# cvjena/semantic-embeddings

Hardware: AMD Instinct MI355X
Metric: retrieval_Mpairs_per_sec (higher is better)
Workload: dtype f32

## Files before the change

semantic-embeddings_amd/csrc/pdist_mfma.hip:

```cpp
#include "se_common.h"
#include <stdlib.h>

namespace se {

typedef float f32x16 __attribute__((ext_vector_type(16)));
typedef float f32x4 __attribute__((ext_vector_type(4)));

constexpr int PD_BM = 128, PD_BN = 128, PD_BK = 64;
constexpr int PD_THREADS = 512;
constexpr int PD_WAVES = PD_THREADS / 64;
constexpr int PD_WROWS = PD_BM / (PD_WAVES / 2);
constexpr int PD_MI = PD_WROWS / 32;
constexpr int PD_LD = PD_BK + 4;
constexpr int PD_SP = PD_BN + 4;
constexpr int PD_SR = (PD_BM * PD_SP <= (PD_BM + PD_BN) * PD_LD) ? PD_BM : PD_BM / 2;
static_assert(PD_SR * PD_SP <= (PD_BM + PD_BN) * PD_LD, "epilogue stage must fit in the operand LDS");
constexpr int PD_GROUP_M = 16;
constexpr int PD_MAX_KB = 16;
constexpr int PD_WGS_PER_CU = 2;
constexpr int PD_F4R = PD_BK / 4;
constexpr int PD_RPP = PD_THREADS / PD_F4R;
constexpr int PD_NLOAD = PD_BM / PD_RPP;
constexpr int64_t PD_MAX_LD = (int64_t)1 << 23;

static_assert(PD_MAX_KB == SE_MAX_KB, "KBlocks capacity");

__device__ __forceinline__ float mask_f(float x, bool keep)
{
    return __uint_as_float(__float_as_uint(x) & (keep ? 0xFFFFFFFFu : 0u));
}

template <bool VEC>
__device__ __forceinline__ void pd_load(float4 (&v)[PD_NLOAD], const float *__restrict__ src, uint32_t ld, int64_t row0,
                                        int64_t nrows, int64_t k0, int64_t kend)
// ... 105 lines not shown
    const uint32_t ldo4 = ldo * 4u;
    float4 cn = make_float4(0.f, 0.f, 0.f, 0.f);
    if (EUC) cn = *(const float4 *)&coln[c4];
#pragma unroll
    for (int p = 0; p < PD_SR / RPP; p++) {
        const int row = p * RPP + r0;
        float4 v = *(const float4 *)&stage[row * PD_SP + c4];
        if (EUC) {
            const float rn = rown[row];
            v = make_float4(fmaf(-2.0f, v.x, rn + cn.x), fmaf(-2.0f, v.y, rn + cn.y), fmaf(-2.0f, v.z, rn + cn.z), fmaf(-2.0f, v.w, rn + cn.w));
        }
        if (dry) { asm volatile("" ::"v"(v.x), "v"(v.y), "v"(v.z), "v"(v.w)); continue; }
        float *dp = (float *)(gb + ((uint32_t)row * ldo4 + (uint32_t)c4 * 4u));
        if (fast) {
            if (nt) __builtin_nontemporal_store((f32x4){v.x, v.y, v.z, v.w}, (f32x4 *)dp);
            else *(float4 *)dp = v;
        } else if (row < nrows) {
            if (c4 < ncols) dp[0] = v.x;
            if (c4 + 1 < ncols) dp[1] = v.y;
            if (c4 + 2 < ncols) dp[2] = v.z;
            if (c4 + 3 < ncols) dp[3] = v.w;
        }
    }
}

template <int METRIC>
__device__ __forceinline__ float pd_finish(float v, float sa, float sb)
{
    if (METRIC == SE_METRIC_COSINE) return -v;
    if (METRIC == SE_METRIC_EUCLID) return (sa + sb) - 2.0f * v;
    return v;
}

constexpr int PDF_VEC_A = 1, PDF_VEC_B = 2, PDF_VEC_O = 4, PDF_NO_STORE = 8, PDF_NO_MFMA = 16, PDF_STAGGER = 32, PDF_PLAIN_ST = 64, PDF_NO_GSTORE = 128;

template <int METRIC, bool MULTI_KB, bool SYM, bool VEC, int EPI>
__global__ __launch_bounds__(PD_THREADS, (PD_WAVES / 4) * PD_WGS_PER_CU) void pdist_kernel(
    const float *__restrict__ A, uint32_t lda, const float *__restrict__ Bm, uint32_t ldb,
    const float *__restrict__ sqa, const float *__restrict__ sqb, int64_t Q, int64_t N, int64_t D,
    KBlocks kbs, int nchunks, float *__restrict__ out, uint32_t ldo, int tiles_m, int tiles_n, int64_t ntiles, int flags,
    unsigned long long *prof, FusedArgs fa)
{
    static_assert(EPI != EPI_GROUPMIN || !SYM, "the sample pass walks the general tile order");
    extern __shared__ __attribute__((aligned(16))) float smem[];
    float *sA = smem;
    float *sB = smem + PD_BM * PD_LD;
    constexpr bool EUC_OUT = METRIC == SE_METRIC_EUCLID && EPI == EPI_STORE;
    [[maybe_unused]] float *sN = smem + (PD_BM + PD_BN) * PD_LD;
    typedef __attribute__((address_space(1))) const void pd_gptr_t;
    typedef __attribute__((address_space(3))) void pd_lptr_t;

    const int64_t b = blockIdx.x, G = gridDim.x;
    const int64_t xcd = b & 7, qq = ntiles >> 3, rr = ntiles & 7;
    const int64_t band_beg = (xcd < rr) ? xcd * (qq + 1) : rr * (qq + 1) + (xcd - rr) * qq;
    const int64_t band_len = qq + (xcd < rr ? 1 : 0);
    const int64_t wg_in_xcd = b >> 3, wgs_per_xcd = (G + 7 - xcd) >> 3;
    const int64_t my_tiles = (band_len > wg_in_xcd) ? (band_len - wg_in_xcd + wgs_per_xcd - 1) / wgs_per_xcd : 0;
    if (my_tiles == 0) return;
    if (flags & PDF_STAGGER) {
        const int slot = (int)((b >> 3) & 3);
        for (int i = 0; i < slot * 2; i++) __builtin_amdgcn_s_sleep(127);
    }

    const int lane = lane_id(), wave = threadIdx.x >> 6;
    const int wm = wave >> 1, wn = wave & 1;
    const int col = lane & 31, hi = lane >> 5;
    const bool vec_o = flags & PDF_VEC_O;
    const bool nt = !(flags & PDF_PLAIN_ST);

    constexpr int NB = 2 * PD_MI;
    f32x16 acc[NB], tot[NB];
#pragma unroll
    for (int j = 0; j < NB; j++)
#pragma unroll
        for (int r = 0; r < 16; r++) { acc[j][r] = 0.f; if (MULTI_KB) tot[j][r] = 0.f; }

    const float *pa = sA + (wm * PD_WROWS + col) * PD_LD + hi * (PD_BK / 2);
    const float *pb0 = sB + (wn * 64 + col) * PD_LD + hi * (PD_BK / 2);
    const float *pb1 = pb0 + 32 * PD_LD;

    float4 ra[PD_NLOAD], rb[PD_NLOAD];
    int64_t m0, n0, k0, kend;
    bool closes_kb;
    pd_tile_coords<SYM>((uint32_t)(band_beg + wg_in_xcd), tiles_m, tiles_n, m0, n0);
    pd_chunk(0, kbs, MULTI_KB, D, k0, kend, closes_kb);
#define PD_FETCH()                              \
    pd_load<VEC>(ra, A, lda, m0, Q, k0, kend);  \
    pd_load<VEC>(rb, Bm, ldb, n0, N, k0, kend);
    PD_FETCH()
    bool first_kb = true;

#ifdef SE_TUNING
    uint64_t t_acc[12] = {0, 0, 0, 0, 0, 0, 0, 0, 0, 0, 0, 0}, t_last = prof ? __builtin_amdgcn_s_memtime() : 0;
#define PD_T(i) if (prof) { const uint64_t now = __builtin_amdgcn_s_memtime(); t_acc[i] += now - t_last; t_last = now; }
#else
#define PD_T(i)
#endif
    const int64_t total = my_tiles * nchunks;
    int c = 0;
    uint32_t tile_i = 0;
    int64_t cur_m0 = m0, cur_n0 = n0;
    int kc = (int)((kend - k0 < PD_BK) ? (kend - k0) : PD_BK);
    bool cur_closes = closes_kb;
    pd_store(sA, ra, (int)((Q - cur_m0 < PD_BM) ? (Q - cur_m0) : PD_BM), kc);
    pd_store(sB, rb, (int)((N - cur_n0 < PD_BN) ? (N - cur_n0) : PD_BN), kc);
    wg_barrier();
#pragma unroll 1
    for (int64_t it = 0; it < total; it++) {
        PD_T(2)
        const bool last_chunk = (c + 1 == nchunks);
        const bool have_next = it + 1 < total;
        if (EUC_OUT && last_chunk) {
            const int w_ = threadIdx.x >> 6;
            if (w_ < (PD_BM + PD_BN) / 64) {
                const int t_ = threadIdx.x & (PD_BM - 1);
                const bool rows_ = w_ < PD_BM / 64;
                const int64_t i_ = rows_ ? (cur_m0 + t_ < Q ? cur_m0 + t_ : Q - 1) : (cur_n0 + t_ < N ? cur_n0 + t_ : N - 1);
                const float *src_ = (rows_ ? sqa : sqb) + i_;
                __builtin_amdgcn_global_load_lds((pd_gptr_t *)src_, (pd_lptr_t *)(sN + w_ * 64), 4, 0, 0);
            }
        }
        if (have_next) {
            const int nc = last_chunk ? 0 : c + 1;
            if (nc == 0) pd_tile_coords<SYM>((uint32_t)(band_beg + wg_in_xcd) + (tile_i + 1u) * (uint32_t)wgs_per_xcd, tiles_m, tiles_n, m0, n0);
            pd_chunk(nc, kbs, MULTI_KB, D, k0, kend, closes_kb);
            PD_FETCH()
        }

        PD_T(3)
        const int steps = (flags & PDF_NO_MFMA) ? 0 : ((kc + 1) >> 1);
        const int full = steps & ~3;
#define PD_STEP(C)                                                                                \
    _Pragma("unroll") for (int mi = 0; mi < PD_MI; mi++) {                                        \
        acc[mi * 2] = __builtin_amdgcn_mfma_f32_32x32x2f32(a4[mi].C, b0.C, acc[mi * 2], 0, 0, 0);         \
        acc[mi * 2 + 1] = __builtin_amdgcn_mfma_f32_32x32x2f32(a4[mi].C, b1.C, acc[mi * 2 + 1], 0, 0, 0); \
    }
#define PD_READ(S)                                                                                \
    float4 a4[PD_MI];                                                                             \
    _Pragma("unroll") for (int mi = 0; mi < PD_MI; mi++) a4[mi] = *(const float4 *)(pa + mi * 32 * PD_LD + (S)); \
    const float4 b0 = *(const float4 *)(pb0 + (S));                                               \
    const float4 b1 = *(const float4 *)(pb1 + (S));
        for (int s = 0; s < full; s += 4) {
            PD_READ(s)
            PD_STEP(x) PD_STEP(y) PD_STEP(z) PD_STEP(w)
        }
        if (steps & 3) {
            PD_READ(full)
            PD_STEP(x)
            if ((steps & 3) > 1) { PD_STEP(y) }
            if ((steps & 3) > 2) { PD_STEP(z) }
        }
#undef PD_READ
#undef PD_STEP

        PD_T(4)
        {
#pragma unroll
            for (int i = 0; i < PD_NLOAD; i++) {
                asm volatile("" : "+v"(ra[i].x), "+v"(ra[i].y), "+v"(ra[i].z), "+v"(ra[i].w));
                asm volatile("" : "+v"(rb[i].x), "+v"(rb[i].y), "+v"(rb[i].z), "+v"(rb[i].w));
            }
        }
        if (MULTI_KB && cur_closes) {
#pragma unroll
            for (int j = 0; j < NB; j++)
#pragma unroll
                for (int r = 0; r < 16; r++) {
                    tot[j][r] = first_kb ? acc[j][r] : (tot[j][r] + acc[j][r]);
                    acc[j][r] = 0.f;
                }
            first_kb = false;
        }

        if (last_chunk) {
            if (EUC_OUT) asm volatile("s_waitcnt vmcnt(0)" ::: "memory");
            if (flags & PDF_NO_STORE) {
#pragma unroll
                for (int j = 0; j < NB; j++)
#pragma unroll
                    for (int r = 0; r < 16; r++) asm volatile("" ::"v"(acc[j][r]));
            } else if (EPI != EPI_STORE) {
                const int rows_here = (int)((Q - cur_m0 < PD_BM) ? (Q - cur_m0) : PD_BM);
                const int cols_here = (int)((N - cur_n0 < PD_BN) ? (N - cur_n0) : PD_BN);
                const bool full_rows = rows_here == PD_BM;
                const int lr0 = wm * PD_WROWS + 4 * hi;
#define PD_FVAL(MI_, J, R)                                                                                                   \
    pd_finish<METRIC>(MULTI_KB ? tot[(MI_) * 2 + (J)][R] : acc[(MI_) * 2 + (J)][R],                                            \
                      METRIC == SE_METRIC_EUCLID ? fsa[((R) & 3) + 4 * ((R) >> 2)] : 0.f, sbq)
                if (EPI == EPI_GROUPMIN) {
#pragma unroll
                    for (int mi = 0; mi < PD_MI; mi++) {
                        float fsa[16];
                        if (METRIC == SE_METRIC_EUCLID) {
#pragma unroll
                            for (int r = 0; r < 16; r++) {
                                const int lr = lr0 + mi * 32 + (r & 3) + 8 * (r >> 2);
                                fsa[r] = sqa[(cur_m0 + (lr < rows_here ? lr : rows_here - 1)) * fa.sqa_stride];
                            }
                        }
#pragma unroll
                        for (int j = 0; j < 2; j++) {
                            const int lc = wn * 64 + j * 32 + col;
                            const bool qok = lc < cols_here;
                            const int64_t qg = cur_n0 + (qok ? lc : cols_here - 1);
                            const float sbq = METRIC == SE_METRIC_EUCLID ? sqb[qg] : 0.f;
                            float m = __builtin_inff();
                            bool any = false;
// ... 176 lines not shown
#pragma unroll
                    for (int h = 0; h < PD_BN / PD_SR; h++) {
                        wg_barrier();
                        PD_T(6)
                        if ((wn * 64) / PD_SR == h) {
#pragma unroll
                            for (int mi = 0; mi < PD_MI; mi++)
#pragma unroll
                                for (int j = 0; j < 2; j++)
#pragma unroll
                                    for (int g = 0; g < 4; g++)
                                        *(float4 *)&smem[(wn * 64 - h * PD_SR + j * 32 + col) * PD_SP + lr0 + mi * 32 + 8 * g] =
                                            make_float4(PD_VAL(mi, j, 4 * g), PD_VAL(mi, j, 4 * g + 1), PD_VAL(mi, j, 4 * g + 2), PD_VAL(mi, j, 4 * g + 3));
                        }
                        PD_T(7)
                        wg_barrier();
                        PD_T(8)
                        pd_stream_rows<EUC_OUT>(smem, out + ((cur_n0 + h * PD_SR) * (int64_t)ldo + cur_m0), ldo, cols_here - h * PD_SR, rows_here, fast, nt,
                                                flags & PDF_NO_GSTORE, sN + PD_BM + h * PD_SR, sN);
                        PD_T(9)
                    }
                }
#undef PD_VAL
            }
#pragma unroll
            for (int j = 0; j < NB; j++)
#pragma unroll
                for (int r = 0; r < 16; r++) acc[j][r] = 0.f;
            first_kb = true;
            PD_T(5)
        }
        wg_barrier();
        PD_T(0)
        if (have_next) {
            cur_m0 = m0; cur_n0 = n0;
            kc = (int)((kend - k0 < PD_BK) ? (kend - k0) : PD_BK);
            cur_closes = closes_kb;
            pd_store(sA, ra, (int)((Q - cur_m0 < PD_BM) ? (Q - cur_m0) : PD_BM), kc);
            pd_store(sB, rb, (int)((N - cur_n0 < PD_BN) ? (N - cur_n0) : PD_BN), kc);
        }
        PD_T(1)
        wg_barrier();
        c = last_chunk ? 0 : c + 1;
        tile_i += last_chunk ? 1u : 0u;
    }
#ifdef SE_TUNING
    if (prof && threadIdx.x == 0)
        for (int i = 0; i < 12; i++) atomicAdd(&prof[i], (unsigned long long)t_acc[i]);
#endif
#undef PD_T
#undef PD_FETCH
}

template <int METRIC, bool MULTI, bool SYM, bool VEC, int EPI = EPI_STORE>
static int launch_pdist3(const float *a, int64_t lda, const float *b, int64_t ldb, const float *sqa, const float *sqb,
                         int64_t q, int64_t n, int64_t d, const KBlocks &kbs, float *out, int64_t ldo, hipStream_t s,
                         const FusedArgs &fa = FusedArgs{nullptr, 0, nullptr, nullptr, nullptr, 0, 1})
{
    const int tiles_m = (int)((q + PD_BM - 1) / PD_BM), tiles_n = (int)((n + PD_BN - 1) / PD_BN);
    const int64_t ntiles = SYM ? ((int64_t)tiles_n * (tiles_n + 1) / 2) : ((int64_t)tiles_m * tiles_n);
    const size_t lds = ((size_t)(PD_BM + PD_BN) * PD_LD + (METRIC == SE_METRIC_EUCLID && EPI == EPI_STORE ? PD_BM + PD_BN : 0)) * sizeof(float);
    if (ntiles >= ((int64_t)1 << 31) || (int64_t)PD_GROUP_M * tiles_n >= ((int64_t)1 << 31) || (SYM && tiles_n > 65535))
        return fail(SE_ERR_UNSUPPORTED, "se_pairwise_dist: %lld output tiles exceed the 32-bit tile counter -- split the call", (long long)ntiles);
    int flags = 0;
    if ((lda % 4 == 0) && ((((uintptr_t)a) & 15) == 0)) flags |= PDF_VEC_A;
    if ((ldb % 4 == 0) && ((((uintptr_t)b) & 15) == 0)) flags |= PDF_VEC_B;
    if ((ldo % 4 == 0) && ((((uintptr_t)out) & 15) == 0)) flags |= PDF_VEC_O;
    flags |= PDF_STAGGER;
    if (kTuning) {
        static const int tune = [] {
            int f = 0;
            if (const char *e = tuning_env("SE_PD_ABLATE")) { const int a = atoi(e); f |= (a & 3) * PDF_NO_STORE; if (a & 4) f |= PDF_NO_GSTORE; }
            if (tuning_env("SE_PD_NOSTAGGER")) f |= 1 << 30;
            if (tuning_env("SE_PD_PLAIN_ST")) f |= PDF_PLAIN_ST;
            return f;
        }();
        flags |= tune & ~(1 << 30);
        if (tune & (1 << 30)) flags &= ~PDF_STAGGER;
    }
    int nchunks = 0;
    for (int i = 0; i < kbs.n; i++) nchunks += (kbs.len[i] + PD_BK - 1) / PD_BK;
    int64_t grid = (int64_t)num_cus() * PD_WGS_PER_CU;
    grid = grid / 8 * 8;
    if (grid > ntiles) grid = ntiles;
    if (grid < 1) grid = 1;
    auto kern = pdist_kernel<METRIC, MULTI, SYM, VEC, EPI>;
    SE_HIP_CHECK(hipFuncSetAttribute((const void *)kern, hipFuncAttributeMaxDynamicSharedMemorySize, (int)lds));
    static const bool profile = tuning_env("SE_PD_PROFILE") != nullptr;
    unsigned long long *prof = nullptr;
    if (profile) {
        SE_HIP_CHECK(hipMalloc((void **)&prof, 12 * sizeof(unsigned long long)));
        SE_HIP_CHECK(hipMemsetAsync(prof, 0, 12 * sizeof(unsigned long long), s));
    }
    hipLaunchKernelGGL(kern, dim3((unsigned)grid), dim3(PD_THREADS), lds, s, a, (uint32_t)lda, b, (uint32_t)ldb, sqa, sqb, q, n,
                       d, kbs, nchunks, out, (uint32_t)ldo, tiles_m, tiles_n, ntiles, flags, prof, fa);
    SE_LAUNCH_CHECK();
    if (profile) {
        unsigned long long h[12];
        SE_HIP_CHECK(hipStreamSynchronize(s));
        SE_HIP_CHECK(hipMemcpy(h, prof, sizeof(h), hipMemcpyDeviceToHost));
        SE_HIP_CHECK(hipFree(prof));
        static const char *names[12] = {"wait-barrier", "stage-operands", "barrier", "prefetch-issue", "mfma", "epilogue-rest",
                                        "epi-barrier-in", "epi-stage-write", "epi-barrier", "epi-stream-out", "-", "-"};
        double tot = 0;
        for (int i = 0; i < 12; i++) tot += (double)h[i];
        fprintf(stderr, "[se_pairwise_dist profile] sym=%d grid=%lld tiles=%lld:", (int)SYM, (long long)grid, (long long)ntiles);
        for (int i = 0; i < 10; i++) fprintf(stderr, " %s %.1f%%", names[i], 100.0 * (double)h[i] / tot);
        fprintf(stderr, "  (%.0f cycles per tile per workgroup)\n", tot / (double)ntiles);
    }
    return SE_OK;
}

template <int METRIC, bool MULTI, bool SYM>
static int launch_pdist2(const float *a, int64_t lda, const float *b, int64_t ldb, const float *sqa, const float *sqb,
                         int64_t q, int64_t n, int64_t d, const KBlocks &kbs, float *out, int64_t ldo, hipStream_t s)
{
    bool vec = (lda % 4 == 0) && ((((uintptr_t)a) & 15) == 0) && (ldb % 4 == 0) && ((((uintptr_t)b) & 15) == 0);
    int64_t beg = 0;
    for (int i = 0; i < kbs.n; i++) { if (beg & 3) vec = false; beg += kbs.len[i]; }
    return vec ? launch_pdist3<METRIC, MULTI, SYM, true>(a, lda, b, ldb, sqa, sqb, q, n, d, kbs, out, ldo, s)
               : launch_pdist3<METRIC, MULTI, SYM, false>(a, lda, b, ldb, sqa, sqb, q, n, d, kbs, out, ldo, s);
}

template <int METRIC>
static int launch_pdist(const float *a, int64_t lda, const float *b, int64_t ldb, const float *sqa, const float *sqb,
                        int64_t q, int64_t n, int64_t d, const KBlocks &kbs, bool multi, float *out, int64_t ldo,
                        hipStream_t s)
{
    const bool sym = (a == b) && (lda == ldb) && (q == n) && (METRIC != SE_METRIC_EUCLID || sqa == sqb) && n > PD_BN;
    if (sym) return multi ? launch_pdist2<METRIC, true, true>(a, lda, b, ldb, sqa, sqb, q, n, d, kbs, out, ldo, s)
                          : launch_pdist2<METRIC, false, true>(a, lda, b, ldb, sqa, sqb, q, n, d, kbs, out, ldo, s);
    return multi ? launch_pdist2<METRIC, true, false>(a, lda, b, ldb, sqa, sqb, q, n, d, kbs, out, ldo, s)
                 : launch_pdist2<METRIC, false, false>(a, lda, b, ldb, sqa, sqb, q, n, d, kbs, out, ldo, s);
// ... 89 lines not shown
```

semantic-embeddings_amd/csrc/rank_rows.hip:

```cpp
#include "se_common.h"
#include <stdlib.h>
#include <atomic>
#include <type_traits>

namespace se {

constexpr int RK_THREADS = 512;
constexpr int RK_WAVES = RK_THREADS / WAVE;
constexpr int RK_ITEMS = 16;
constexpr int RK_TILE = RK_THREADS * RK_ITEMS;
constexpr int RK_WCHUNK = RK_TILE / RK_WAVES;
constexpr int RK_NB = 256;

struct RankLds {
    uint32_t gbase[4][RK_NB];
    uint32_t wcnt[RK_WAVES][RK_NB];
    uint32_t tile_start[RK_NB];
    uint32_t wave_tot[RK_WAVES];
    uint32_t tkeys[RK_TILE];
    uint32_t tidx[RK_TILE];
};

__device__ __forceinline__ uint32_t wave_excl_scan(uint32_t v, uint32_t &total)
{
// ... 399 lines not shown
    constexpr int BITS = HWORD ? RR_HW_BITS : 8;
    constexpr int NB = 1 << BITS;
    constexpr int NPASS = (32 + BITS - 1) / BITS;
    constexpr int CNT_WORDS = HWORD ? NB / 2 : NB;
    constexpr bool WIDE = HWORD && ((size_t)RR_THREADS * ITEMS * sizeof(uint16_t) >= (size_t)RR_WAVES * RR_WIDE_WORDS * sizeof(uint32_t));
    constexpr bool IMG = WIDE && VAR == 3;
    constexpr bool RAWKEYS = IMG || (WIDE && VAR == 2);
    static_assert(VAR != 3 || (WIDE && ITEMS <= RR_IMG_MAX_ITEMS && !SEG), "image path: long-row instantiations with room for the tag plane");
    uint32_t *wcnt = reinterpret_cast<uint32_t *>(rr_raw);
    uint32_t *wave_tot = reinterpret_cast<uint32_t *>(rr_raw + rr_region0_bytes<ITEMS, HWORD, VAR>());
    uint16_t *xbuf = reinterpret_cast<uint16_t *>(wave_tot + 32);
    [[maybe_unused]] uint8_t *tagb = rr_raw;
    [[maybe_unused]] uint32_t *wlist = reinterpret_cast<uint32_t *>(rr_raw + (size_t)RR_THREADS * ITEMS + 32);
    [[maybe_unused]] uint32_t *ictl = wave_tot + 24;
    const int tid = threadIdx.x, lane = tid & 63, wave = tid >> 6;
    [[maybe_unused]] const int wave_s = __builtin_amdgcn_readfirstlane(wave);
    const int wpos0 = wave * (ITEMS * WAVE) + lane;
    const uint32_t xb = lds_off(xbuf);
    const uint32_t rb = xb + 2u * (uint32_t)wpos0;
    static_assert(rr_region0_bytes<ITEMS, HWORD, VAR>() % 16 == 0 && (ITEMS * WAVE * sizeof(uint16_t)) % 8 == 0, "transposed reads need 8-byte aligned addresses");
    [[maybe_unused]] const uint32_t rt = xb + 2u * (uint32_t)(wave * (ITEMS * WAVE)) + rr_tr_lane_off((uint32_t)lane);
#define RR_DST(IR) (xb + (((IR) & 0xFFFFu) << 1))
    auto row_ptr = [&](int64_t v) -> const float * {
        if constexpr (SEG) return pdist + (v >> seg.shift) * ldp + (v & ((1 << seg.shift) - 1)) * (int64_t)seg.seg_n;
        else return pdist + v * ldp;
    };
    auto row_len = [&](int64_t v) -> int {
        if constexpr (SEG) {
            const int rest = N - (int)(v & ((1 << seg.shift) - 1)) * seg.seg_n;
            return rest < seg.seg_n ? rest : seg.seg_n;
        } else return N;
    };
    uint32_t t_acc[12] = {0, 0, 0, 0, 0, 0, 0, 0, 0, 0, 0, 0}, t_last = PROF ? (uint32_t)__builtin_amdgcn_s_memtime() : 0;
#define RR_T(i) if constexpr (PROF) { const uint32_t now = (uint32_t)__builtin_amdgcn_s_memtime(); t_acc[i] += now - t_last; t_last = now; } else { asm volatile("" ::: "memory"); __builtin_amdgcn_sched_barrier(0); }

    uint32_t key[ITEMS], ir[ITEMS];
    __amdgpu_buffer_rsrc_t ld_rsrc;
    uint32_t ld_voff = 0;
    uint64_t ring[RR_RING / 2];
#define RR_LOAD_ONE(DROW, WPOS, S, NN)                                                                               \
    {                                                                                                                 \
        if ((S) % 16 == 0) {                                                                                          \
            if ((S) == 0) {                                                                                           \
                ld_rsrc = __builtin_amdgcn_make_buffer_rsrc(const_cast<float *>(DROW), 0, (NN) * 4, 0x00020000);     \
                ld_voff = (uint32_t)(WPOS) * 4u;                                                                      \
            } else ld_voff += 4096u;                                                                                  \
            opaque(ld_voff);                                                                                          \
        }                                                                                                             \
        key[S] = (uint32_t)__builtin_amdgcn_raw_buffer_load_b32(ld_rsrc, (int)ld_voff + ((S) % 16) * 256, 0, 0);      \
    }
#define RR_CANON(NN)                                                                                                  \
    {                                                                                                                 \
        int wpos_ = wpos0;                                                                                            \
        opaque(wpos_);                                                                                                \
        const uint32_t pk_ = rr_pad_key((uint32_t)wpos_ & 63u);                                                       \
        _Pragma("unroll") for (int s = 0; s < ITEMS; s++) {                                                           \
            const int pos = wpos_ + s * WAVE;                                                                         \
            key[s] = rr_key(key[s], pos >= (NN), pk_ + (ITEMS <= 88 ? (uint32_t)((((s >> 3) & 7) << 17) | ((s & 7) << 6)) : 0u));  \
        }                                                                                                             \
    }
#define RR_PREFETCH_NEXT_ROW() RR_PREFETCH_NEXT_ROW_IF(end >= 32 && more)
#define RR_PREFETCH_NEXT_ROW_IF(COND) \
    if (COND) { \
                const char *nrow = (const char *)row_ptr(row + gridDim.x); \
                const uint32_t row_bytes = (uint32_t)row_len(row + gridDim.x) * 4u; \
                for (uint32_t off = (uint32_t)tid * 128u; off < row_bytes; off += RR_THREADS * 128u) \
// ... 620 lines not shown
                    const int j = j0 + u * RR_THREADS * 4;
                    v[u] = *reinterpret_cast<const uint2 *>(xbuf + (j < N ? j : 0));
                }
#pragma unroll
                for (int u = 0; u < RR_WO; u++) {
                    const int j = j0 + u * RR_THREADS * 4;
                    if (j >= N) break;
                    const int e0 = v[u].x & 0xFFFFu, e1 = v[u].x >> 16, e2 = v[u].y & 0xFFFFu, e3 = v[u].y >> 16;
                    if (vec_ok && j + 3 < N) {
                        __builtin_nontemporal_store((rr_i32x4){e0, e1, e2, e3}, reinterpret_cast<rr_i32x4 *>(o + j));
                    } else {
                        o[j] = e0;
                        if (j + 1 < N) o[j + 1] = e1;
                        if (j + 2 < N) o[j + 2] = e2;
                        if (j + 3 < N) o[j + 3] = e3;
                    }
                }
            }
        }
        RR_T(7)
        if constexpr (!RAWKEYS) RR_CANON(n_next)
        if constexpr (PROF) {
            _Pragma("unroll") for (int s = 0; s < ITEMS; s++) opaque(key[s]);
        }
        if constexpr (!IMG)
            asm volatile("s_waitcnt vmcnt(0)" : "+v"(pf_sink) : : "memory");
        RR_T(0)
        if constexpr (IMG) {
            if (img_fail) {
                if (img_level == 0) { img_pen0 = img_pen0 ? (img_pen0 < 16 ? 2 * img_pen0 : 32) : 1; img_skip0 = img_pen0; }
                else { img_pen1 = img_pen1 ? (img_pen1 < 16 ? 2 * img_pen1 : 32) : 1; img_skip1 = img_pen1; }
                img_level++;
                img_again = true;
            } else {
                if (two) { if (img_level == 0) img_pen0 = 0; else img_pen1 = 0; }
                img_again = false;
                row += gridDim.x;
            }
        } else row += gridDim.x;
    }
    if (PROF && tid == 0)
    {
        for (int i = 0; i < 12; i++) atomicAdd(&prof[i], (unsigned long long)t_acc[i]);
    }
#undef RR_T
}

}

using namespace se;

static size_t rank_idx_bytes(int idx) { return idx == 2 ? 2 : (idx ? 8 : 4); }

static int rank_grid(int64_t q)
{
    const int64_t g = 512;
    return (int)(q < g ? q : g);
}

static int64_t rank_npad(int64_t n) { return (n + 63) / 64 * 64; }

static bool rank_use_tiled(int64_t n)
{
    static const bool force = tuning_env("SE_RANK_TILED") != nullptr;
    return force || n > RR_MAX_N;
}

__global__ __launch_bounds__(256) void rank_skew_detect_kernel(const float *__restrict__ pdist, int64_t ldp, int64_t Q, int N,
                                                               int shift, int two_ok, uint32_t *__restrict__ flag)
{
    constexpr int NBIN = 4096;
    __shared__ uint32_t hist[NBIN], hash_hist[NBIN];
    __shared__ uint32_t best, row_max[3], row_below[3], repeats;
    for (int i = threadIdx.x; i < NBIN; i += 256) { hist[i] = 0; hash_hist[i] = 0; }
    if (threadIdx.x == 0) { best = 0; repeats = 0; }
    if (threadIdx.x < 3) { row_max[threadIdx.x] = 0; row_below[threadIdx.x] = 0; }
    wg_barrier();
// ... 40 lines not shown
        *flag = (two && distinct) ? 2u : (skewed ? 1u : (((two_ok & 2) && distinct) ? 3u : 0u));
    }
}

struct Resident { hipError_t err; int64_t grid; };
static Resident rank_resident(const void *kern, size_t lds)
{
    hipError_t e = hipFuncSetAttribute(kern, hipFuncAttributeMaxDynamicSharedMemorySize, (int)lds);
    int dev = 0, occ = 0;
    hipDeviceProp_t prop;
    if (e == hipSuccess) e = hipGetDevice(&dev);
    if (e == hipSuccess) e = hipGetDeviceProperties(&prop, dev);
    if (e == hipSuccess) e = hipOccupancyMaxActiveBlocksPerMultiprocessor(&occ, kern, RR_THREADS, lds);
    if (e != hipSuccess) return {e, 0};
    return {hipSuccess, (int64_t)(prop.multiProcessorCount > 0 ? prop.multiProcessorCount : 256) * (occ > 0 ? occ : 1)};
}

template <int ITEMS, bool HW, int VAR>
static int launch_rank_reg_variant(const float *pdist, int64_t ldp, int64_t q, int n, void *rank, int idx64, int64_t ldr,
                                   const uint32_t *skew_flag, hipStream_t s)
{
    const size_t lds = rr_region0_bytes<ITEMS, HW, VAR>() + 32 * sizeof(uint32_t) + (size_t)RR_THREADS * ITEMS * sizeof(uint16_t);
    static_assert(rr_region0_bytes<ITEMS, HW, VAR>() + 32 * sizeof(uint32_t) + (size_t)RR_THREADS * ITEMS * sizeof(uint16_t) <= 160 * 1024, "LDS of one CU");
    static const bool profile = tuning_env("SE_RR_PROFILE") != nullptr;
    auto kern = (kTuning && profile) ? rank_rows_reg_kernel<ITEMS, kTuning && (ITEMS == 98), HW, VAR> : rank_rows_reg_kernel<ITEMS, false, HW, VAR>;
    static const Resident res = rank_resident((const void *)kern, lds);
    if (res.err != hipSuccess) return fail(SE_ERR_HIP, "se_rank_rows: kernel set-up failed: %s", hipGetErrorString(res.err));
    int64_t grid = res.grid;
    if (grid > q) grid = q;
    const size_t esz = rank_idx_bytes(idx64);
    const int vec_ok = ((((uintptr_t)rank) & 15) == 0) && ((ldr * esz) % 16 == 0);
    unsigned long long *prof = nullptr;
    if (profile && ITEMS == 98) {
        SE_HIP_CHECK(hipMalloc((void **)&prof, 36 * sizeof(unsigned long long)));
        SE_HIP_CHECK(hipMemsetAsync(prof, 0, 36 * sizeof(unsigned long long), s));
    }
    hipLaunchKernelGGL(kern, dim3((unsigned)grid), dim3(RR_THREADS), lds, s, pdist, ldp, q, n, rank, ldr, idx64, vec_ok, prof, skew_flag, RankSeg{0, 0, nullptr, 0});
    SE_LAUNCH_CHECK();
    if (prof) {
        unsigned long long h[36];
        SE_HIP_CHECK(hipStreamSynchronize(s));
        SE_HIP_CHECK(hipMemcpy(h, prof, sizeof(h), hipMemcpyDeviceToHost));
        SE_HIP_CHECK(hipFree(prof));
        static const char *names[12] = {"load", "rank", "scan", "dest", "idx-write", "idx-read", "key-exchange", "write-out", "image-map|window-map", "tag-scan|window-max", "repair|window-barrier-1", "window-count|scan-barrier"};
        double tot = 0;
        for (int i = 0; i < 12; i++) tot += (double)h[i];
        if (tot > 0) {
            fprintf(stderr, "[se_rank_rows profile] ITEMS=%d hw=%d peel=%d grid=%lld:", ITEMS, (int)HW, VAR, (long long)grid);
            for (int i = 0; i < 12; i++) fprintf(stderr, " %s %.1f%%", names[i], 100.0 * (double)h[i] / tot);
            fprintf(stderr, "  (%.0f cycles per row; wave 0 of every workgroup, timestamps behind the phases' own barriers)", tot / (double)q);
            fprintf(stderr, "\n");
        }
    }
    return SE_OK;
}

template <int ITEMS>
static int launch_rank_reg(const float *pdist, int64_t ldp, int64_t q, int n, void *rank, int idx64, int64_t ldr, bool hw, void *scratch,
                           hipStream_t s)
{
    if (!hw) return launch_rank_reg_variant<ITEMS, false, 0>(pdist, ldp, q, n, rank, idx64, ldr, nullptr, s);
    constexpr bool wide = (size_t)RR_THREADS * ITEMS * sizeof(uint16_t) >= (size_t)RR_WAVES * RR_WIDE_WORDS * sizeof(uint32_t);
    constexpr bool two_ok = wide;
    constexpr bool img_ok = wide && ITEMS <= RR_IMG_MAX_ITEMS;
    static const char *force = tuning_env("SE_RANK_PEEL");
    if (force || !scratch) {
        if (force && force[0] == '1') return launch_rank_reg_variant<ITEMS, true, 1>(pdist, ldp, q, n, rank, idx64, ldr, nullptr, s);
        if (force && force[0] == '2' && two_ok) return launch_rank_reg_variant<ITEMS, true, two_ok ? 2 : 0>(pdist, ldp, q, n, rank, idx64, ldr, nullptr, s);
        if (force && force[0] == '3' && img_ok) return launch_rank_reg_variant<ITEMS, true, img_ok ? 3 : 0>(pdist, ldp, q, n, rank, idx64, ldr, nullptr, s);
        return launch_rank_reg_variant<ITEMS, true, 0>(pdist, ldp, q, n, rank, idx64, ldr, nullptr, s);
    }
    uint32_t *flag = (uint32_t *)scratch + 16;
    const int top_shift = wide ? 20 : 2 * RR_HW_BITS;
    hipLaunchKernelGGL(rank_skew_detect_kernel, dim3(1), dim3(256), 0, s, pdist, ldp, q, n, top_shift, (two_ok ? 1 : 0) | (img_ok ? 2 : 0), flag);
    SE_LAUNCH_CHECK();
// ... 657 lines not shown
```

semantic-embeddings_amd/csrc/se_common.h:

```cpp
#pragma once
#include <hip/hip_runtime.h>
#include <stdint.h>
#include <stdio.h>
#include <stdarg.h>
#include <stdlib.h>
#include <type_traits>

#include "../../include/sehip.h"

namespace se {

char *err_buf();
int fail(int code, const char *fmt, ...);

__attribute__((visibility("hidden"))) int num_cus();

__attribute__((visibility("hidden"))) void launch_mean(const float *v, int64_t n, float *out, hipStream_t s);

void phase_mark(const char *name, hipStream_t s);
bool phase_timing_on();
void phase_note_counters(const unsigned *dev_counters, long long rows, hipStream_t s);

#define SE_HIP_CHECK(expr)                                                                     \
    do {                                                                                       \
        hipError_t e__ = (expr);                                                               \
        if (e__ != hipSuccess)                                                                 \
            return se::fail(SE_ERR_HIP, "%s failed: %s (%s:%d)", #expr, hipGetErrorString(e__), \
                            __FILE__, __LINE__);                                               \
    } while (0)

#define SE_LAUNCH_CHECK()                                                                      \
    do {                                                                                       \
        hipError_t e__ = hipGetLastError();                                                    \
        if (e__ != hipSuccess)                                                                 \
            return se::fail(SE_ERR_HIP, "kernel launch failed: %s (%s:%d)",                    \
                            hipGetErrorString(e__), __FILE__, __LINE__);                       \
    } while (0)

constexpr int WAVE = 64;

#ifdef SE_TUNING
inline const char *tuning_env(const char *name) { return getenv(name); }
constexpr bool kTuning = true;
#else
inline const char *tuning_env(const char *) { return nullptr; }
constexpr bool kTuning = false;
#endif

__device__ __forceinline__ void wg_barrier()
{
    asm volatile("s_waitcnt lgkmcnt(0)" ::: "memory");
    __syncthreads();
}

__device__ __forceinline__ uint32_t canon_key(float f)
{
    uint32_t u = __float_as_uint(f);
    if (f != f) return 0xFFFFFFFFu;
    if (u == 0x80000000u) u = 0u;
    return (u & 0x80000000u) ? ~u : (u | 0x80000000u);
}

__device__ __forceinline__ float bf16_to_f32(uint16_t h) { return __uint_as_float(((uint32_t)h) << 16); }

__device__ __forceinline__ uint16_t f32_to_bf16(float f)
{
    uint32_t u = __float_as_uint(f);
    if (f != f) return (uint16_t)((u >> 16) | 0x40);
    u += 0x7FFFu + ((u >> 16) & 1u);
    return (uint16_t)(u >> 16);
}

template <class T>
__device__ __forceinline__ T wave_sum(T v)
{
#pragma unroll
    for (int off = 32; off > 0; off >>= 1) v += __shfl_xor(v, off, 64);
    return v;
}
// ... 164 lines not shown
```

Measured before the change: 242,500.

## Add dynamic work-stealing tile queue to pdist store kernel

Replaces the static per-XCD tile striding in the pairwise-distance store kernel with an atomic per-XCD queue. Workgroups claim tiles from their own band and steal from the fullest other band when it runs dry, and the next claim is overlapped with the MFMA loop. A host-side pool of queue buffers, guarded by events and a mutex, supplies the counters, with a fallback to the static schedule under graph capture or when a buffer is still busy. The aim is to remove tail imbalance across workgroups, at the cost of atomic traffic, an extra barrier and host locking per launch; per-workgroup profiling dumps are also added.

```diff
diff --git a/semantic-embeddings_amd/csrc/pdist_mfma.hip b/semantic-embeddings_amd/csrc/pdist_mfma.hip
--- a/semantic-embeddings_amd/csrc/pdist_mfma.hip
+++ b/semantic-embeddings_amd/csrc/pdist_mfma.hip
@@ -1,5 +1,6 @@
 #include "se_common.h"
 #include <stdlib.h>
+#include <mutex>
 
 namespace se {
 
@@ -171,21 +172,53 @@
     return v;
 }
 
+constexpr int PDQ_WORDS = 16;
+constexpr uint32_t PD_NO_TILE = 0xFFFFFFFFu;
+__device__ __forceinline__ uint32_t pdq_band_len(int k, uint32_t qq, uint32_t rr) { return qq + ((uint32_t)k < rr ? 1u : 0u); }
+__device__ __forceinline__ uint32_t pdq_band_beg(int k, uint32_t qq, uint32_t rr) { return (uint32_t)k < rr ? (uint32_t)k * (qq + 1u) : rr * (qq + 1u) + ((uint32_t)k - rr) * qq; }
+__device__ __forceinline__ uint32_t pdq_resolve(uint32_t *queue, uint32_t got, int own, uint32_t qq, uint32_t rr)
+{
+    if (got < pdq_band_len(own, qq, rr)) return pdq_band_beg(own, qq, rr) + got;
+    for (;;) {
+        uint32_t c[8];
+#pragma unroll
+        for (int k = 0; k < 8; k++) c[k] = __hip_atomic_load(&queue[k], __ATOMIC_RELAXED, __HIP_MEMORY_SCOPE_AGENT);
+        int best = -1;
+        uint32_t most = 0;
+#pragma unroll
+        for (int k = 0; k < 8; k++) {
+            const uint32_t len = pdq_band_len(k, qq, rr), left = c[k] < len ? len - c[k] : 0u;
+            if (left > most) { most = left; best = k; }
+        }
+        if (best < 0) return PD_NO_TILE;
+        const uint32_t g = atomicAdd(&queue[best], 1u);
+        if (g < pdq_band_len(best, qq, rr)) return pdq_band_beg(best, qq, rr) + g;
+    }
+}
+__device__ __forceinline__ void pdq_leave(uint32_t *queue)
+{
+    if (atomicAdd(&queue[8], 1u) == gridDim.x - 1u)
+        for (int k = 0; k <= 8; k++) atomicExch(&queue[k], 0u);
+}
+
 constexpr int PDF_VEC_A = 1, PDF_VEC_B = 2, PDF_VEC_O = 4, PDF_NO_STORE = 8, PDF_NO_MFMA = 16, PDF_STAGGER = 32, PDF_PLAIN_ST = 64, PDF_NO_GSTORE = 128;
 
-template <int METRIC, bool MULTI_KB, bool SYM, bool VEC, int EPI>
+template <int METRIC, bool MULTI_KB, bool SYM, bool VEC, int EPI, bool DYN = false>
 __global__ __launch_bounds__(PD_THREADS, (PD_WAVES / 4) * PD_WGS_PER_CU) void pdist_kernel(
     const float *__restrict__ A, uint32_t lda, const float *__restrict__ Bm, uint32_t ldb,
     const float *__restrict__ sqa, const float *__restrict__ sqb, int64_t Q, int64_t N, int64_t D,
     KBlocks kbs, int nchunks, float *__restrict__ out, uint32_t ldo, int tiles_m, int tiles_n, int64_t ntiles, int flags,
-    unsigned long long *prof, FusedArgs fa)
+    unsigned long long *prof, FusedArgs fa, uint32_t *queue)
 {
     static_assert(EPI != EPI_GROUPMIN || !SYM, "the sample pass walks the general tile order");
+    static_assert(!DYN || EPI == EPI_STORE, "the fused top-k passes keep the static lists");
     extern __shared__ __attribute__((aligned(16))) float smem[];
     float *sA = smem;
     float *sB = smem + PD_BM * PD_LD;
     constexpr bool EUC_OUT = METRIC == SE_METRIC_EUCLID && EPI == EPI_STORE;
     [[maybe_unused]] float *sN = smem + (PD_BM + PD_BN) * PD_LD;
+    constexpr bool dyn = DYN;
+    [[maybe_unused]] uint32_t *sQ = reinterpret_cast<uint32_t *>(smem + (PD_BM + PD_BN) * PD_LD + (EUC_OUT ? PD_BM + PD_BN : 0));
     typedef __attribute__((address_space(1))) const void pd_gptr_t;
     typedef __attribute__((address_space(3))) void pd_lptr_t;
 
@@ -194,8 +227,24 @@
     const int64_t band_beg = (xcd < rr) ? xcd * (qq + 1) : rr * (qq + 1) + (xcd - rr) * qq;
     const int64_t band_len = qq + (xcd < rr ? 1 : 0);
     const int64_t wg_in_xcd = b >> 3, wgs_per_xcd = (G + 7 - xcd) >> 3;
-    const int64_t my_tiles = (band_len > wg_in_xcd) ? (band_len - wg_in_xcd + wgs_per_xcd - 1) / wgs_per_xcd : 0;
+    const int64_t my_tiles = dyn ? 1 : ((band_len > wg_in_xcd) ? (band_len - wg_in_xcd + wgs_per_xcd - 1) / wgs_per_xcd : 0);
     if (my_tiles == 0) return;
+    [[maybe_unused]] const int qx = (int)blockIdx.x & 7;
+    [[maybe_unused]] const uint32_t qlen = (uint32_t)(ntiles >> 3), qrem = (uint32_t)ntiles & 7u;
+    uint32_t t_cur = (uint32_t)(band_beg + wg_in_xcd), t_nxt = PD_NO_TILE;
+    if constexpr (dyn) {
+        if (threadIdx.x == 0) {
+            uint32_t t0 = pdq_resolve(queue, atomicAdd(&queue[qx], 1u), qx, qlen, qrem), t1 = PD_NO_TILE;
+            if (t0 != PD_NO_TILE) t1 = pdq_resolve(queue, atomicAdd(&queue[qx], 1u), qx, qlen, qrem);
+            sQ[0] = t0;
+            sQ[1] = t1;
+            if (t0 == PD_NO_TILE) pdq_leave(queue);
+        }
+        wg_barrier();
+        t_cur = (uint32_t)__builtin_amdgcn_readfirstlane((int)sQ[0]);
+        t_nxt = (uint32_t)__builtin_amdgcn_readfirstlane((int)sQ[1]);
+        if (t_cur == PD_NO_TILE) return;
+    }
     if (flags & PDF_STAGGER) {
         const int slot = (int)((b >> 3) & 3);
         for (int i = 0; i < slot * 2; i++) __builtin_amdgcn_s_sleep(127);
@@ -221,7 +270,7 @@
     float4 ra[PD_NLOAD], rb[PD_NLOAD];
     int64_t m0, n0, k0, kend;
     bool closes_kb;
-    pd_tile_coords<SYM>((uint32_t)(band_beg + wg_in_xcd), tiles_m, tiles_n, m0, n0);
+    pd_tile_coords<SYM>(t_cur, tiles_m, tiles_n, m0, n0);
     pd_chunk(0, kbs, MULTI_KB, D, k0, kend, closes_kb);
 #define PD_FETCH()                              \
     pd_load<VEC>(ra, A, lda, m0, Q, k0, kend);  \
@@ -231,6 +280,8 @@
 
 #ifdef SE_TUNING
     uint64_t t_acc[12] = {0, 0, 0, 0, 0, 0, 0, 0, 0, 0, 0, 0}, t_last = prof ? __builtin_amdgcn_s_memtime() : 0;
+    const uint64_t wgs_t0 = t_last, wgs_rt0 = prof ? __builtin_amdgcn_s_memrealtime() : 0;
+    uint32_t wgs_partial = 0, wgs_diag = 0, wgs_done = 0;
 #define PD_T(i) if (prof) { const uint64_t now = __builtin_amdgcn_s_memtime(); t_acc[i] += now - t_last; t_last = now; }
 #else
 #define PD_T(i)
@@ -245,10 +296,11 @@
     pd_store(sB, rb, (int)((N - cur_n0 < PD_BN) ? (N - cur_n0) : PD_BN), kc);
     wg_barrier();
 #pragma unroll 1
-    for (int64_t it = 0; it < total; it++) {
+    for (int64_t it = 0; dyn || it < total; it++) {
         PD_T(2)
         const bool last_chunk = (c + 1 == nchunks);
-        const bool have_next = it + 1 < total;
+        const bool have_next = dyn ? (!last_chunk || t_nxt != PD_NO_TILE) : (it + 1 < total);
+        const bool claim = dyn && last_chunk && t_nxt != PD_NO_TILE;
         if (EUC_OUT && last_chunk) {
             const int w_ = threadIdx.x >> 6;
             if (w_ < (PD_BM + PD_BN) / 64) {
@@ -261,10 +313,12 @@
         }
         if (have_next) {
             const int nc = last_chunk ? 0 : c + 1;
-            if (nc == 0) pd_tile_coords<SYM>((uint32_t)(band_beg + wg_in_xcd) + (tile_i + 1u) * (uint32_t)wgs_per_xcd, tiles_m, tiles_n, m0, n0);
+            if (nc == 0) pd_tile_coords<SYM>(dyn ? t_nxt : (uint32_t)(band_beg + wg_in_xcd) + (tile_i + 1u) * (uint32_t)wgs_per_xcd, tiles_m, tiles_n, m0, n0);
             pd_chunk(nc, kbs, MULTI_KB, D, k0, kend, closes_kb);
             PD_FETCH()
         }
+        [[maybe_unused]] uint32_t got = 0;
+        if (dyn && claim && threadIdx.x == 0) got = atomicAdd(&queue[qx], 1u);
 
         PD_T(3)
         const int steps = (flags & PDF_NO_MFMA) ? 0 : ((kc + 1) >> 1);
@@ -299,6 +353,10 @@
                 asm volatile("" : "+v"(ra[i].x), "+v"(ra[i].y), "+v"(ra[i].z), "+v"(ra[i].w));
                 asm volatile("" : "+v"(rb[i].x), "+v"(rb[i].y), "+v"(rb[i].z), "+v"(rb[i].w));
             }
+            if constexpr (dyn) {
+                asm volatile("" : "+v"(got));
+                if (claim && threadIdx.x == 0) sQ[1] = pdq_resolve(queue, got, qx, qlen, qrem);
+            }
         }
         if (MULTI_KB && cur_closes) {
 #pragma unroll
@@ -312,6 +370,13 @@
         }
 
         if (last_chunk) {
+#ifdef SE_TUNING
+            if (prof) {
+                wgs_done++;
+                wgs_partial += (Q - cur_m0 < PD_BM || N - cur_n0 < PD_BN) ? 1u : 0u;
+                wgs_diag += (SYM && cur_m0 == cur_n0) ? 1u : 0u;
+            }
+#endif
             if (EUC_OUT) asm volatile("s_waitcnt vmcnt(0)" ::: "memory");
             if (flags & PDF_NO_STORE) {
 #pragma unroll
@@ -554,6 +619,10 @@
         }
         wg_barrier();
         PD_T(0)
+        if constexpr (dyn) {
+            if (!have_next) break;
+            if (claim) t_nxt = (uint32_t)__builtin_amdgcn_readfirstlane((int)sQ[1]);
+        }
         if (have_next) {
             cur_m0 = m0; cur_n0 = n0;
             kc = (int)((kend - k0 < PD_BK) ? (kend - k0) : PD_BK);
@@ -566,12 +635,58 @@
         c = last_chunk ? 0 : c + 1;
         tile_i += last_chunk ? 1u : 0u;
     }
+    if (dyn && threadIdx.x == 0) pdq_leave(queue);
 #ifdef SE_TUNING
-    if (prof && threadIdx.x == 0)
+    if (prof && threadIdx.x == 0) {
         for (int i = 0; i < 12; i++) atomicAdd(&prof[i], (unsigned long long)t_acc[i]);
+        wgs_write(prof + 12 + (size_t)blockIdx.x * WGS_WORDS, wgs_t0, wgs_rt0, wgs_done, wgs_partial, wgs_diag);
+    }
 #endif
 #undef PD_T
 #undef PD_FETCH
+}
+
+constexpr int PDQ_BLOCKS = 32, PDQ_DEVICES = 64;
+struct PdQueues {
+    uint32_t *dev = nullptr;
+    hipEvent_t done[PDQ_BLOCKS] = {};
+    bool used[PDQ_BLOCKS] = {};
+    unsigned next = 0;
+    bool failed = false;
+};
+static std::mutex pdq_mu;
+static PdQueues pdq_state[PDQ_DEVICES];
+
+static uint32_t *pdq_take(hipStream_t s, hipEvent_t *done)
+{
+    hipStreamCaptureStatus cap = hipStreamCaptureStatusNone;
+    int dev = 0;
+    if (hipStreamIsCapturing(s, &cap) != hipSuccess || cap != hipStreamCaptureStatusNone || hipGetDevice(&dev) != hipSuccess || dev < 0 ||
+        dev >= PDQ_DEVICES) {
+        (void)hipGetLastError();
+        return nullptr;
+    }
+    PdQueues &q = pdq_state[dev];
+    if (q.failed) return nullptr;
+    if (!q.dev) {
+        bool ok = hipMalloc((void **)&q.dev, (size_t)PDQ_BLOCKS * PDQ_WORDS * sizeof(uint32_t)) == hipSuccess;
+        ok = ok && hipMemset(q.dev, 0, (size_t)PDQ_BLOCKS * PDQ_WORDS * sizeof(uint32_t)) == hipSuccess;
+        for (int i = 0; ok && i < PDQ_BLOCKS; i++) ok = hipEventCreateWithFlags(&q.done[i], hipEventDisableTiming) == hipSuccess;
+        if (!ok) {
+            (void)hipGetLastError();
+            q.failed = true;
+            return nullptr;
+        }
+    }
+    const unsigned b = q.next % PDQ_BLOCKS;
+    if (q.used[b] && hipEventQuery(q.done[b]) != hipSuccess) {
+        (void)hipGetLastError();
+        return nullptr;
+    }
+    q.next++;
+    q.used[b] = true;
+    *done = q.done[b];
+    return q.dev + (size_t)b * PDQ_WORDS;
 }
 
 template <int METRIC, bool MULTI, bool SYM, bool VEC, int EPI = EPI_STORE>
@@ -581,7 +696,7 @@
 {
     const int tiles_m = (int)((q + PD_BM - 1) / PD_BM), tiles_n = (int)((n + PD_BN - 1) / PD_BN);
     const int64_t ntiles = SYM ? ((int64_t)tiles_n * (tiles_n + 1) / 2) : ((int64_t)tiles_m * tiles_n);
-    const size_t lds = ((size_t)(PD_BM + PD_BN) * PD_LD + (METRIC == SE_METRIC_EUCLID && EPI == EPI_STORE ? PD_BM + PD_BN : 0)) * sizeof(float);
+    const size_t lds = ((size_t)(PD_BM + PD_BN) * PD_LD + (METRIC == SE_METRIC_EUCLID && EPI == EPI_STORE ? PD_BM + PD_BN : 0) + (EPI == EPI_STORE ? 4 : 0)) * sizeof(float);
     if (ntiles >= ((int64_t)1 << 31) || (int64_t)PD_GROUP_M * tiles_n >= ((int64_t)1 << 31) || (SYM && tiles_n > 65535))
         return fail(SE_ERR_UNSUPPORTED, "se_pairwise_dist: %lld output tiles exceed the 32-bit tile counter -- split the call", (long long)ntiles);
     int flags = 0;
@@ -608,19 +723,40 @@
     if (grid < 1) grid = 1;
     auto kern = pdist_kernel<METRIC, MULTI, SYM, VEC, EPI>;
     SE_HIP_CHECK(hipFuncSetAttribute((const void *)kern, hipFuncAttributeMaxDynamicSharedMemorySize, (int)lds));
+    if constexpr (EPI == EPI_STORE)
+        SE_HIP_CHECK(hipFuncSetAttribute((const void *)pdist_kernel<METRIC, MULTI, SYM, VEC, EPI, true>, hipFuncAttributeMaxDynamicSharedMemorySize, (int)lds));
     static const bool profile = tuning_env("SE_PD_PROFILE") != nullptr;
     unsigned long long *prof = nullptr;
     if (profile) {
-        SE_HIP_CHECK(hipMalloc((void **)&prof, 12 * sizeof(unsigned long long)));
-        SE_HIP_CHECK(hipMemsetAsync(prof, 0, 12 * sizeof(unsigned long long), s));
+        SE_HIP_CHECK(hipMalloc((void **)&prof, (12 + (size_t)grid * WGS_WORDS) * sizeof(unsigned long long)));
+        SE_HIP_CHECK(hipMemsetAsync(prof, 0, (12 + (size_t)grid * WGS_WORDS) * sizeof(unsigned long long), s));
+    }
+    uint32_t *queue = nullptr;
+    hipEvent_t queue_done = nullptr;
+    std::unique_lock<std::mutex> queue_lock(pdq_mu, std::defer_lock);
+    static const bool pin_static = tuning_env("SE_PD_STATIC") != nullptr;
+    if (EPI == EPI_STORE && !pin_static) {
+        queue_lock.lock();
+        queue = pdq_take(s, &queue_done);
+        if (queue) kern = pdist_kernel<METRIC, MULTI, SYM, VEC, EPI, EPI == EPI_STORE>;
     }
     hipLaunchKernelGGL(kern, dim3((unsigned)grid), dim3(PD_THREADS), lds, s, a, (uint32_t)lda, b, (uint32_t)ldb, sqa, sqb, q, n,
-                       d, kbs, nchunks, out, (uint32_t)ldo, tiles_m, tiles_n, ntiles, flags, prof, fa);
+                       d, kbs, nchunks, out, (uint32_t)ldo, tiles_m, tiles_n, ntiles, flags, prof, fa, queue);
     SE_LAUNCH_CHECK();
+    if (queue) SE_HIP_CHECK(hipEventRecord(queue_done, s));
+    if (queue_lock.owns_lock()) queue_lock.unlock();
     if (profile) {
         unsigned long long h[12];
         SE_HIP_CHECK(hipStreamSynchronize(s));
         SE_HIP_CHECK(hipMemcpy(h, prof, sizeof(h), hipMemcpyDeviceToHost));
+#ifdef SE_TUNING
+        {
+            unsigned long long *wg = (unsigned long long *)malloc((size_t)grid * WGS_WORDS * sizeof(unsigned long long));
+            if (wg && hipMemcpy(wg, prof + 12, (size_t)grid * WGS_WORDS * sizeof(unsigned long long), hipMemcpyDeviceToHost) == hipSuccess)
+                wgs_dump(EPI == EPI_STORE ? (SYM ? "pdist_sym" : "pdist_general") : "pdist_fused", wg, (long long)grid);
+            free(wg);
+        }
+#endif
         SE_HIP_CHECK(hipFree(prof));
         static const char *names[12] = {"wait-barrier", "stage-operands", "barrier", "prefetch-issue", "mfma", "epilogue-rest",
                                         "epi-barrier-in", "epi-stage-write", "epi-barrier", "epi-stream-out", "-", "-"};
diff --git a/semantic-embeddings_amd/csrc/rank_rows.hip b/semantic-embeddings_amd/csrc/rank_rows.hip
--- a/semantic-embeddings_amd/csrc/rank_rows.hip
+++ b/semantic-embeddings_amd/csrc/rank_rows.hip
@@ -455,6 +455,8 @@
         } else return N;
     };
     uint32_t t_acc[12] = {0, 0, 0, 0, 0, 0, 0, 0, 0, 0, 0, 0}, t_last = PROF ? (uint32_t)__builtin_amdgcn_s_memtime() : 0;
+    [[maybe_unused]] const uint64_t wgs_t0 = PROF ? __builtin_amdgcn_s_memtime() : 0, wgs_rt0 = PROF ? __builtin_amdgcn_s_memrealtime() : 0;
+    [[maybe_unused]] uint32_t wgs_rows = 0, wgs_giveups = 0;
 #define RR_T(i) if constexpr (PROF) { const uint32_t now = (uint32_t)__builtin_amdgcn_s_memtime(); t_acc[i] += now - t_last; t_last = now; } else { asm volatile("" ::: "memory"); __builtin_amdgcn_sched_barrier(0); }
 
     uint32_t key[ITEMS], ir[ITEMS];
@@ -1141,17 +1143,22 @@
                 else { img_pen1 = img_pen1 ? (img_pen1 < 16 ? 2 * img_pen1 : 32) : 1; img_skip1 = img_pen1; }
                 img_level++;
                 img_again = true;
+                if constexpr (PROF) wgs_giveups++;
             } else {
                 if (two) { if (img_level == 0) img_pen0 = 0; else img_pen1 = 0; }
                 img_again = false;
                 row += gridDim.x;
-            }
-        } else row += gridDim.x;
-    }
+                if constexpr (PROF) wgs_rows++;
+            }
+        } else { row += gridDim.x; if constexpr (PROF) wgs_rows++; }
+    }
+#ifdef SE_TUNING
     if (PROF && tid == 0)
     {
         for (int i = 0; i < 12; i++) atomicAdd(&prof[i], (unsigned long long)t_acc[i]);
-    }
+        wgs_write(prof + 36 + (size_t)blockIdx.x * WGS_WORDS, wgs_t0, wgs_rt0, wgs_rows, wgs_giveups, 0u);
+    }
+#endif
 #undef RR_T
 }
 
@@ -1258,8 +1265,8 @@
     const int vec_ok = ((((uintptr_t)rank) & 15) == 0) && ((ldr * esz) % 16 == 0);
     unsigned long long *prof = nullptr;
     if (profile && ITEMS == 98) {
-        SE_HIP_CHECK(hipMalloc((void **)&prof, 36 * sizeof(unsigned long long)));
-        SE_HIP_CHECK(hipMemsetAsync(prof, 0, 36 * sizeof(unsigned long long), s));
+        SE_HIP_CHECK(hipMalloc((void **)&prof, (36 + (size_t)grid * WGS_WORDS) * sizeof(unsigned long long)));
+        SE_HIP_CHECK(hipMemsetAsync(prof, 0, (36 + (size_t)grid * WGS_WORDS) * sizeof(unsigned long long), s));
     }
     hipLaunchKernelGGL(kern, dim3((unsigned)grid), dim3(RR_THREADS), lds, s, pdist, ldp, q, n, rank, ldr, idx64, vec_ok, prof, skew_flag, RankSeg{0, 0, nullptr, 0});
     SE_LAUNCH_CHECK();
@@ -1267,6 +1274,14 @@
         unsigned long long h[36];
         SE_HIP_CHECK(hipStreamSynchronize(s));
         SE_HIP_CHECK(hipMemcpy(h, prof, sizeof(h), hipMemcpyDeviceToHost));
+#ifdef SE_TUNING
+        if (h[0] + h[1] + h[7] > 0) {
+            unsigned long long *wg = (unsigned long long *)malloc((size_t)grid * WGS_WORDS * sizeof(unsigned long long));
+            if (wg && hipMemcpy(wg, prof + 36, (size_t)grid * WGS_WORDS * sizeof(unsigned long long), hipMemcpyDeviceToHost) == hipSuccess)
+                wgs_dump(VAR == 3 ? "rank_rows_image" : (VAR == 2 ? "rank_rows_window" : (VAR == 1 ? "rank_rows_peel" : "rank_rows_plain")), wg, (long long)grid);
+            free(wg);
+        }
+#endif
         SE_HIP_CHECK(hipFree(prof));
         static const char *names[12] = {"load", "rank", "scan", "dest", "idx-write", "idx-read", "key-exchange", "write-out", "image-map|window-map", "tag-scan|window-max", "repair|window-barrier-1", "window-count|scan-barrier"};
         double tot = 0;
diff --git a/semantic-embeddings_amd/csrc/se_common.h b/semantic-embeddings_amd/csrc/se_common.h
--- a/semantic-embeddings_amd/csrc/se_common.h
+++ b/semantic-embeddings_amd/csrc/se_common.h
@@ -45,6 +45,34 @@
 #else
 inline const char *tuning_env(const char *) { return nullptr; }
 constexpr bool kTuning = false;
+#endif
+
+constexpr int WGS_WORDS = 8;
+#ifdef SE_TUNING
+__device__ __forceinline__ void wgs_write(unsigned long long *rec, uint64_t t_in, uint64_t rt_in, uint32_t done, uint32_t partial, uint32_t diag)
+{
+    rec[0] = t_in;
+    rec[1] = __builtin_amdgcn_s_memtime();
+    rec[2] = rt_in;
+    rec[3] = __builtin_amdgcn_s_memrealtime();
+    rec[4] = done;
+    rec[5] = partial;
+    rec[6] = diag;
+    rec[7] = (unsigned long long)(__builtin_amdgcn_s_getreg((3 << 11) | 20) & 0xF) |
+             ((unsigned long long)(uint32_t)__builtin_amdgcn_s_getreg((31 << 11) | 4) << 8);
+}
+inline void wgs_dump(const char *kernel, const unsigned long long *h, long long grid)
+{
+    const char *path = getenv("SE_WG_DUMP");
+    FILE *f = path ? fopen(path, "a") : nullptr;
+    if (!f) return;
+    fprintf(f, "launch %s grid %lld\n", kernel, grid);
+    for (long long b = 0; b < grid; b++) {
+        const unsigned long long *r = h + b * WGS_WORDS;
+        fprintf(f, "wg %lld %llu %llu %llu %llu %llu %llu %llu %llu\n", b, r[0], r[1], r[2], r[3], r[4], r[5], r[6], r[7]);
+    }
+    fclose(f);
+}
 #endif
 
 __device__ __forceinline__ void wg_barrier()
```

Measured after the change: 242,400 (median of 2 runs). About the same (-0.0%).
